# Roboy/gym-roboy

Hardware: AMD Instinct MI355X
Metric: env-steps/sec, MsjRobot (3-DOF/8-tendon) batched rollout (higher is better)
Workload: dtype f32

## Files before the change

gym_roboy_amd/csrc/msj_math.hpp:

```cpp
#pragma once
#include "rtc_compat.hpp"

#if defined(__HIPCC__)
#define RB_HD __host__ __device__ __forceinline__
#else
#define RB_HD inline
#endif


namespace rb {

template <typename T> struct Fast;
template <> struct Fast<double> {
    static RB_HD void sincos(double x, double &s, double &c) { s = ::sin(x); c = ::cos(x); }
    static RB_HD double exp(double x) { return ::exp(x); }
    static RB_HD double exp2(double x) { return ::exp2(x); }
    static RB_HD double rsqrt(double x) { return 1.0 / ::sqrt(x); }
    static RB_HD double rcp(double x) { return 1.0 / x; }
};
template <> struct Fast<float> {
    static RB_HD void sincos(float x, float &s, float &c) {
#if defined(__HIP_DEVICE_COMPILE__)
        s = __sinf(x); c = __cosf(x);
#else
        s = ::sinf(x); c = ::cosf(x);
#endif
    }
    static RB_HD float exp(float x) {
#if defined(__HIP_DEVICE_COMPILE__)
        return __expf(x);
#else
        return ::expf(x);
#endif
    }
    static RB_HD float exp2(float x) {
#if defined(__HIP_DEVICE_COMPILE__)
        return __builtin_amdgcn_exp2f(x);
#else
        return ::exp2f(x);
#endif
    }
    static RB_HD float rsqrt(float x) {
#if defined(__HIP_DEVICE_COMPILE__)
        return __builtin_amdgcn_rsqf(x);
#else
        return 1.0f / ::sqrtf(x);
#endif
    }
    static RB_HD float rcp(float x) {
#if defined(__HIP_DEVICE_COMPILE__)
        return __builtin_amdgcn_rcpf(x);
#else
        return 1.0f / x;
#endif
    }
};

template <typename T> RB_HD T tmin(T a, T b) {
#if defined(__HIP_DEVICE_COMPILE__)
    if constexpr (std::is_same<T, float>::value) return __builtin_fminf(a, b);
#endif
    return a < b ? a : b;
}
template <typename T> RB_HD T tmax(T a, T b) {
#if defined(__HIP_DEVICE_COMPILE__)
    if constexpr (std::is_same<T, float>::value) return __builtin_fmaxf(a, b);
#endif
    return a > b ? a : b;
}
template <typename T> RB_HD T tclamp(T x, T lo, T hi) {
#if defined(__HIP_DEVICE_COMPILE__)
    if constexpr (std::is_same<T, float>::value) return __builtin_amdgcn_fmed3f(x, lo, hi);
#endif
    return tmin(tmax(x, lo), hi);
}

template <typename T>
struct alignas(64) MsjTendon {
    T A[3];
    T Bv[3];
    T B2[3];
    T ab2;
    T il0s;
    T elcs;
    T ksg;
    T fmaxv;
    T pad[2];
};

template <typename T>
struct TendonUnits {
    T lc;
    T vl0;
    T fmax;
    T pad;
};

template <typename T>
struct TendonReading { T length, rate, activation, force; };

template <typename T, int NT>
struct MsjConst {
    MsjTendon<T> ten[NT];
    T IO[6];
    T mc[3];
    T g[3];
    T arm[3], damp[3], qlo[3], qhi[3], qdmax[3];
    T kps;
    T pe_k2s;
    T inv_pe_den;
    T fv_c1l, fv_c2l;
    T fv_c2s;
    T fv_k;
    T h;
    int32_t nsub;
    int32_t simple;
    int32_t nt;
};

template <typename T, int NT>
struct SpArray {
    const T *v;
    RB_HD T operator()(int k) const { return v[k]; }
};

struct NominalBody {
    template <typename T> RB_HD T mass(T x) const { return x; }
    template <typename T> RB_HD T damping(int, T x) const { return x; }
};

template <typename T, int NT>
struct MsjModel {
    using C = MsjConst<T, NT>;

    struct Frame {
        T s0, c0, s1, c1, s2, c2;
        T r00, r01, r02, r10, r11, r12, r20, r21, r22;
        T wx, wy, wz;
    };

    static RB_HD Frame frame(const T q[3], const T qd[3]) {
        Frame f;
        Fast<T>::sincos(q[0], f.s0, f.c0);
        Fast<T>::sincos(q[1], f.s1, f.c1);
        Fast<T>::sincos(q[2], f.s2, f.c2);
        f.r00 = f.c1 * f.c2; f.r01 = -f.c1 * f.s2; f.r02 = f.s1;
        f.r10 = f.c0 * f.s2 + f.s0 * f.s1 * f.c2; f.r11 = f.c0 * f.c2 - f.s0 * f.s1 * f.s2; f.r12 = -f.s0 * f.c1;
        f.r20 = f.s0 * f.s2 - f.c0 * f.s1 * f.c2; f.r21 = f.s0 * f.c2 + f.c0 * f.s1 * f.s2; f.r22 = f.c0 * f.c1;
        f.wx = f.r00 * qd[0] + f.s2 * qd[1];
        f.wy = f.r01 * qd[0] + f.c2 * qd[1];
        f.wz = f.r02 * qd[0] + qd[2];
        return f;
    }

    static RB_HD void tendon(const C &c, const Frame &f, const MsjTendon<T> &t, T u, T &tx, T &ty, T &tz) {
        const T ax = f.r00 * t.A[0] + f.r10 * t.A[1] + f.r20 * t.A[2];
        const T ay = f.r01 * t.A[0] + f.r11 * t.A[1] + f.r21 * t.A[2];
        const T az = f.r02 * t.A[0] + f.r12 * t.A[1] + f.r22 * t.A[2];
        const T d2 = ax * t.B2[0] + (ay * t.B2[1] + (az * t.B2[2] + t.ab2));
        const T mx = ay * t.Bv[2] - az * t.Bv[1];
        const T my = az * t.Bv[0] - ax * t.Bv[2];
        const T mz = ax * t.Bv[1] - ay * t.Bv[0];
        tendon_force(c, f, t, u, d2, mx, my, mz, tx, ty, tz);
    }

    static RB_HD void tendon_force(const C &c, const Frame &f, const MsjTendon<T> &t, T u, T d2, T mx, T my, T mz,
                                   T &tx, T &ty, T &tz) {
        const T inv = Fast<T>::rsqrt(d2);
        const T v = (f.wx * mx + f.wy * my + f.wz * mz) * inv;
        const T es = (d2 * inv) * t.il0s + t.elcs;
        const T act = tclamp(c.kps * es - u, T(0), T(1));
        const T fl = Fast<T>::exp2(-(es * es));
        const T vp = tmax(v, T(0)), p = tclamp(v + T(1), T(0), T(1));
        const T num = c.fv_c1l * vp + p;
        const T den = c.fv_c2l * vp + (c.fv_c2s * p + c.fv_k);
        const T rden = Fast<T>::rcp(den);
        const T fpe = tmax(Fast<T>::exp2(c.pe_k2s * es) * c.inv_pe_den - c.inv_pe_den, T(0));
        const T Fs = (t.fmaxv * inv) * ((act * fl) * num * rden + fpe);
        tx -= Fs * mx; ty -= Fs * my; tz -= Fs * mz;
    }

    static RB_HD TendonReading<T> tendon_state(const C &c, const Frame &f, const MsjTendon<T> &t, const TendonUnits<T> &pu, T u) {
        return tendon_state_sel(c, f, t, pu, u, true);
    }
    static RB_HD TendonReading<T> tendon_state_sel(const C &c, const Frame &f, const MsjTendon<T> &t, const TendonUnits<T> &pu, T u,
                                                   bool want_force) {
        const T ax = f.r00 * t.A[0] + f.r10 * t.A[1] + f.r20 * t.A[2];
        const T ay = f.r01 * t.A[0] + f.r11 * t.A[1] + f.r21 * t.A[2];
        const T az = f.r02 * t.A[0] + f.r12 * t.A[1] + f.r22 * t.A[2];
        const T d2 = ax * t.B2[0] + (ay * t.B2[1] + (az * t.B2[2] + t.ab2));
        const T mx = ay * t.Bv[2] - az * t.Bv[1];
        const T my = az * t.Bv[0] - ax * t.Bv[2];
        const T mz = ax * t.Bv[1] - ay * t.Bv[0];
        const T inv = Fast<T>::rsqrt(d2);
        const T v = (f.wx * mx + f.wy * my + f.wz * mz) * inv;
        const T dl = d2 * inv;
        const T es = dl * t.il0s + t.elcs;
        const T act = tclamp(c.kps * es - u, T(0), T(1));
        TendonReading<T> r;
        r.length = dl + pu.lc;
        r.rate = v * pu.vl0;
        r.activation = act;
        r.force = T(0);
        if (want_force) {
            const T fl = Fast<T>::exp2(-(es * es));
            const T vp = tmax(v, T(0)), p = tclamp(v + T(1), T(0), T(1));
            const T num = c.fv_c1l * vp + p;
            const T den = c.fv_c2l * vp + (c.fv_c2s * p + c.fv_k);
            const T rden = Fast<T>::rcp(den);
            const T fpe = tmax(Fast<T>::exp2(c.pe_k2s * es) * c.inv_pe_den - c.inv_pe_den, T(0));
            r.force = pu.fmax * ((act * fl) * num * rden + fpe);
        }
        return r;
    }

    static RB_HD MsjTendon<T> scaled_tendon(const MsjTendon<T> &t, T fscale) {
        MsjTendon<T> s = t;
        s.fmaxv = t.fmaxv * fscale;
        return s;
    }

    static RB_HD T prescale(const C &c, int k, T setpoint) { return c.ten[k].ksg * setpoint; }

    template <typename BP> static RB_HD T bmass(const BP *bp, T x) {
        if constexpr (std::is_same<BP, NominalBody>::value) return x; else return bp->mass(x);
    }
    template <typename BP> static RB_HD T bdamp(const BP *bp, int j, T x) {
        if constexpr (std::is_same<BP, NominalBody>::value) return x; else return bp->damping(j, x);
    }
    template <typename BP = NominalBody>
    static RB_HD void rigid_body(const C &c, const Frame &f, const T qd[3], T tx, T ty, T tz, T qdd[3], const BP *bp = nullptr) {
        const T r00 = f.r00, r01 = f.r01, r02 = f.r02, s2 = f.s2, c2 = f.c2;
        const T Ixx = bmass(bp, c.IO[0]), Iyy = bmass(bp, c.IO[1]), Izz = bmass(bp, c.IO[2]);
        const T z0x = -f.s1 * c2 * qd[1] - f.c1 * s2 * qd[2];
        const T z0y = f.s1 * s2 * qd[1] - f.c1 * c2 * qd[2];
        const T z0z = f.c1 * qd[1];
        const T bx = z0x * qd[0] + c2 * qd[2] * qd[1];
        const T by = z0y * qd[0] - s2 * qd[2] * qd[1];
        const T bz = z0z * qd[0];
        T m00, m01, m02, m11, m12, m22, vx, vy, vz;
        if (c.simple) {
            const T a0x = Ixx * r00, a0y = Iyy * r01, a0z = Izz * r02;
            const T a1x = Ixx * s2, a1y = Iyy * c2;
            m00 = r00 * a0x + r01 * a0y + r02 * a0z + c.arm[0];
            m01 = s2 * a0x + c2 * a0y;
            m02 = a0z;
            m11 = s2 * a1x + c2 * a1y + c.arm[1];
            m12 = T(0);
            m22 = Izz + c.arm[2];
            const T hx = Ixx * f.wx, hy = Iyy * f.wy, hz = Izz * f.wz;
            const T nx = Ixx * bx + (f.wy * hz - f.wz * hy);
            const T ny = Iyy * by + (f.wz * hx - f.wx * hz);
            const T nz = Izz * bz + (f.wx * hy - f.wy * hx);
            const T k = bmass(bp, c.mc[2]) * c.g[2];
            vx = tx - k * f.r21 - nx;
            vy = ty + k * f.r20 - ny;
            vz = tz - nz;
        } else {
            const T Ixy = bmass(bp, c.IO[3]), Ixz = bmass(bp, c.IO[4]), Iyz = bmass(bp, c.IO[5]);
            const T a0x = Ixx * r00 + Ixy * r01 + Ixz * r02;
            const T a0y = Ixy * r00 + Iyy * r01 + Iyz * r02;
            const T a0z = Ixz * r00 + Iyz * r01 + Izz * r02;
            const T a1x = Ixx * s2 + Ixy * c2;
            const T a1y = Ixy * s2 + Iyy * c2;
            const T a1z = Ixz * s2 + Iyz * c2;
            m00 = r00 * a0x + r01 * a0y + r02 * a0z + c.arm[0];
            m01 = s2 * a0x + c2 * a0y;
            m02 = a0z;
            m11 = s2 * a1x + c2 * a1y + c.arm[1];
            m12 = a1z;
            m22 = Izz + c.arm[2];
            const T hx = a0x * qd[0] + a1x * qd[1] + Ixz * qd[2];
            const T hy = a0y * qd[0] + a1y * qd[1] + Iyz * qd[2];
            const T hz = a0z * qd[0] + a1z * qd[1] + Izz * qd[2];
            const T nx = Ixx * bx + Ixy * by + Ixz * bz + (f.wy * hz - f.wz * hy);
            const T ny = Ixy * bx + Iyy * by + Iyz * bz + (f.wz * hx - f.wx * hz);
            const T nz = Ixz * bx + Iyz * by + Izz * bz + (f.wx * hy - f.wy * hx);
            const T gx = r00 * c.g[0] + f.r10 * c.g[1] + f.r20 * c.g[2];
            const T gy = r01 * c.g[0] + f.r11 * c.g[1] + f.r21 * c.g[2];
            const T gz = r02 * c.g[0] + f.r12 * c.g[1] + f.r22 * c.g[2];
            vx = tx + (bmass(bp, c.mc[1]) * gz - bmass(bp, c.mc[2]) * gy) - nx;
            vy = ty + (bmass(bp, c.mc[2]) * gx - bmass(bp, c.mc[0]) * gz) - ny;
            vz = tz + (bmass(bp, c.mc[0]) * gy - bmass(bp, c.mc[1]) * gx) - nz;
        }
        const T t0 = r00 * vx + r01 * vy + r02 * vz - bdamp(bp, 0, c.damp[0]) * qd[0];
        const T t1 = s2 * vx + c2 * vy - bdamp(bp, 1, c.damp[1]) * qd[1];
        const T t2 = vz - bdamp(bp, 2, c.damp[2]) * qd[2];
        const T k00 = m11 * m22 - m12 * m12;
        const T k01 = m02 * m12 - m01 * m22;
        const T k02 = m01 * m12 - m02 * m11;
        const T k11 = m00 * m22 - m02 * m02;
        const T k12 = m01 * m02 - m00 * m12;
        const T k22 = m00 * m11 - m01 * m01;
        const T idet = Fast<T>::rcp(m00 * k00 + m01 * k01 + m02 * k02);
        qdd[0] = (k00 * t0 + k01 * t1 + k02 * t2) * idet;
        qdd[1] = (k01 * t0 + k11 * t1 + k12 * t2) * idet;
        qdd[2] = (k02 * t0 + k12 * t1 + k22 * t2) * idet;
    }

    template <int UNROLL, typename SP>
    struct AccelAllTendons {
        const C &c;
        const SP &sp;
        RB_HD void operator()(const T q[3], const T qd[3], T qdd[3]) const {
            const Frame f = frame(q, qd);
            T tx = T(0), ty = T(0), tz = T(0);
            if (UNROLL == 0) {
#pragma unroll 1
                for (int k = 0; k < c.nt; ++k) tendon(c, f, c.ten[k], sp(k), tx, ty, tz);
            } else {
                constexpr int U = UNROLL > 0 ? UNROLL : 1;
#pragma unroll U
                for (int k = 0; k < NT; ++k) tendon(c, f, c.ten[k], sp(k), tx, ty, tz);
            }
            rigid_body(c, f, qd, tx, ty, tz, qdd);
        }
    };

    template <int MIRROR> static RB_HD T mirror_sign(int j) { return (j == 2 || j == MIRROR) ? T(-1) : T(1); }
    static RB_HD void half_torque(const C &c, const Frame &f, const T u[4], T &tx, T &ty, T &tz) {
        tx = T(0); ty = T(0); tz = T(0);
#pragma unroll
        for (int k = 0; k < 4; ++k) {
            tendon(c, f, c.ten[k], u[k], tx, ty, tz);
#if defined(__HIP_DEVICE_COMPILE__)
            __builtin_amdgcn_sched_barrier(0);
#endif
        }
    }
    template <int MIRROR>
    static RB_HD void mirror_combine(T &tx, T &ty, T &tz, T px, T py, T pz) {
        tx = MIRROR == 0 ? tx - px : tx + px;
        ty = MIRROR == 0 ? ty + py : ty - py;
        tz = tz - pz;
    }

    static RB_HD void sat(const C &c, const T v[3], T out[3]) {
#pragma unroll
        for (int j = 0; j < 3; ++j) out[j] = tclamp(v[j], -c.qdmax[j], c.qdmax[j]);
    }

    static RB_HD bool limit(const C &c, T q[3], T qd[3]) {
        bool ok = true;
#pragma unroll
        for (int j = 0; j < 3; ++j) {
            const bool over = q[j] > c.qhi[j], under = q[j] < c.qlo[j];
            qd[j] = tclamp(qd[j], under ? T(0) : -c.qdmax[j], over ? T(0) : c.qdmax[j]);
            q[j] = tclamp(q[j], c.qlo[j], c.qhi[j]);
            ok = ok && !(over || under);
        }
        return ok;
    }

    template <int INTEG, typename ACCEL>
    static RB_HD bool integrate(const C &c, T q[3], T qd[3], const ACCEL &accel) {
        bool feasible = true;
        const T h = c.h;
        for (int sub = 0; sub < c.nsub; ++sub) {
            if (INTEG == 0) {
                T a[3];
                accel(q, qd, a);
#pragma unroll
                for (int j = 0; j < 3; ++j) {
                    qd[j] = tclamp(qd[j] + h * a[j], -c.qdmax[j], c.qdmax[j]);
                    q[j] = q[j] + h * qd[j];
                }
            } else {
                T k1q[3], k1v[3], k2q[3], k2v[3], k3q[3], k3v[3], k4q[3], k4v[3], qs[3], vs[3];
                const T hh = T(0.5) * h;
                sat(c, qd, k1q);
                accel(q, k1q, k1v);
#pragma unroll
                for (int j = 0; j < 3; ++j) { qs[j] = q[j] + hh * k1q[j]; vs[j] = qd[j] + hh * k1v[j]; }
                sat(c, vs, k2q);
                accel(qs, k2q, k2v);
#pragma unroll
                for (int j = 0; j < 3; ++j) { qs[j] = q[j] + hh * k2q[j]; vs[j] = qd[j] + hh * k2v[j]; }
                sat(c, vs, k3q);
                accel(qs, k3q, k3v);
#pragma unroll
                for (int j = 0; j < 3; ++j) { qs[j] = q[j] + h * k3q[j]; vs[j] = qd[j] + h * k3v[j]; }
                sat(c, vs, k4q);
                accel(qs, k4q, k4v);
                const T h6 = h * T(1.0 / 6.0);
#pragma unroll
                for (int j = 0; j < 3; ++j) {
                    q[j] = q[j] + h6 * (k1q[j] + T(2) * k2q[j] + T(2) * k3q[j] + k4q[j]);
                    qd[j] = qd[j] + h6 * (k1v[j] + T(2) * k2v[j] + T(2) * k3v[j] + k4v[j]);
                }
            }
            feasible = limit(c, q, qd) && feasible;
        }
        return feasible;
    }

    template <int INTEG, typename ACCEL>
    static RB_HD bool integrate_acc(const C &c, T q[3], T qd[3], const ACCEL &accel) {
        if (INTEG == 0) return integrate<0>(c, q, qd, accel);
        bool feasible = true;
        const T h = c.h, h6 = c.h * T(1.0 / 6.0);
        for (int sub = 0; sub < c.nsub; ++sub) {
            T aq[3] = {T(0), T(0), T(0)}, av[3] = {T(0), T(0), T(0)}, qs[3], vs[3];
#pragma unroll
            for (int j = 0; j < 3; ++j) { qs[j] = q[j]; vs[j] = qd[j]; }
#pragma unroll 1
            for (int stage = 0; stage < 4; ++stage) {
                T kq[3], kv[3];
                sat(c, vs, kq);
                accel(qs, kq, kv);
                const T w = (stage == 0 || stage == 3) ? T(1) : T(2);
                const T a = stage < 2 ? T(0.5) * h : h;
#pragma unroll
                for (int j = 0; j < 3; ++j) {
                    aq[j] += w * kq[j]; av[j] += w * kv[j];
                    qs[j] = q[j] + a * kq[j]; vs[j] = qd[j] + a * kv[j];
                }
            }
#pragma unroll
            for (int j = 0; j < 3; ++j) { q[j] = q[j] + h6 * aq[j]; qd[j] = qd[j] + h6 * av[j]; }
            feasible = limit(c, q, qd) && feasible;
        }
        return feasible;
    }

    struct AccelPinned {
        const C &c;
        const T *u;
        RB_HD void operator()(const T q[3], const T qd[3], T qdd[3]) const {
            const Frame f = frame(q, qd);
            T tx = T(0), ty = T(0), tz = T(0);
#pragma unroll
            for (int k = 0; k < NT; ++k) {
                tendon(c, f, c.ten[k], u[k], tx, ty, tz);
#if defined(__HIP_DEVICE_COMPILE__)
                __builtin_amdgcn_sched_barrier(0);
#endif
            }
            rigid_body(c, f, qd, tx, ty, tz, qdd);
        }
    };

    struct Routing { T d2, mx, my, mz; };
    static RB_HD Routing routing(const Frame &f, const MsjTendon<T> &t) {
        const T ax = f.r00 * t.A[0] + f.r10 * t.A[1] + f.r20 * t.A[2];
        const T ay = f.r01 * t.A[0] + f.r11 * t.A[1] + f.r21 * t.A[2];
        const T az = f.r02 * t.A[0] + f.r12 * t.A[1] + f.r22 * t.A[2];
        Routing r;
        r.d2 = ax * t.B2[0] + (ay * t.B2[1] + (az * t.B2[2] + t.ab2));
        r.mx = ay * t.Bv[2] - az * t.Bv[1];
        r.my = az * t.Bv[0] - ax * t.Bv[2];
        r.mz = ax * t.Bv[1] - ay * t.Bv[0];
        return r;
    }
    struct Strain { T v, es, fl, pe; };
    static RB_HD Strain strain(const C &c, const Frame &f, const MsjTendon<T> &t, const Routing &r, T inv) {
        Strain s;
        s.v = (f.wx * r.mx + f.wy * r.my + f.wz * r.mz) * inv;
        s.es = (r.d2 * inv) * t.il0s + t.elcs;
        s.fl = Fast<T>::exp2(-(s.es * s.es));
        s.pe = Fast<T>::exp2(c.pe_k2s * s.es);
        return s;
    }
    struct Hill { T afn, rden; };
    static RB_HD Hill hill(const C &c, const Strain &s, T u) {
        const T act = tclamp(c.kps * s.es - u, T(0), T(1));
        const T vp = tmax(s.v, T(0)), p = tclamp(s.v + T(1), T(0), T(1));
        const T num = c.fv_c1l * vp + p;
        const T den = c.fv_c2l * vp + (c.fv_c2s * p + c.fv_k);
        Hill h;
        h.rden = Fast<T>::rcp(den);
        h.afn = (act * s.fl) * num;
        return h;
    }
    static RB_HD void torque(const C &c, const MsjTendon<T> &t, const Routing &r, T inv, const Strain &s, const Hill &h,
                             T &tx, T &ty, T &tz) {
        const T fpe = tmax(s.pe * c.inv_pe_den - c.inv_pe_den, T(0));
        const T Fs = (t.fmaxv * inv) * (h.afn * h.rden + fpe);
        tx -= Fs * r.mx; ty -= Fs * r.my; tz -= Fs * r.mz;
    }
    static RB_HD void pin() {
#if defined(__HIP_DEVICE_COMPILE__)
        __builtin_amdgcn_sched_barrier(0);
#endif
    }
    static RB_HD void tendon_pair(const C &c, const Frame &f, const MsjTendon<T> &ta, const MsjTendon<T> &tb, T ua, T ub,
                                  T &tx, T &ty, T &tz) {
        const Routing ra = routing(f, ta);
        pin();
        const T ia = Fast<T>::rsqrt(ra.d2);
        const Routing rb_ = routing(f, tb);
        pin();
        const T ib = Fast<T>::rsqrt(rb_.d2);
        const Strain sa = strain(c, f, ta, ra, ia);
        pin();
        const Hill ha = hill(c, sa, ua);
        const Strain sb = strain(c, f, tb, rb_, ib);
        pin();
        torque(c, ta, ra, ia, sa, ha, tx, ty, tz);
        const Hill hb = hill(c, sb, ub);
        pin();
        torque(c, tb, rb_, ib, sb, hb, tx, ty, tz);
        pin();
    }
    template <typename SP>
    struct AccelPaired {
        const C &c;
        const SP &sp;
        RB_HD void operator()(const T q[3], const T qd[3], T qdd[3]) const {
            static_assert(NT % 2 == 0, "tendons in pairs");
            const Frame f = frame(q, qd);
            T tx = T(0), ty = T(0), tz = T(0);
#pragma unroll
            for (int k = 0; k < NT; k += 2) {
                const T ua = sp(k), ub = sp(k + 1);
                tendon_pair(c, f, c.ten[k], c.ten[k + 1], ua, ub, tx, ty, tz);
            }
            rigid_body(c, f, qd, tx, ty, tz, qdd);
        }
    };
    static constexpr int RS = 9;
    template <int INTEG>
    static RB_HD bool step_rs(const C &c, T q[3], T qd[3], const T u[NT]) {
        return integrate_acc<INTEG>(c, q, qd, AccelPinned{c, u});
    }

    template <int INTEG, typename SP>
    static RB_HD bool step_rs_paired(const C &c, T q[3], T qd[3], const SP &sp) {
        return integrate_acc<INTEG>(c, q, qd, AccelPaired<SP>{c, sp});
    }

    template <int INTEG, int UNROLL, typename SP>
    static RB_HD bool step_sp(const C &c, T q[3], T qd[3], const SP &sp) {
        return integrate<INTEG>(c, q, qd, AccelAllTendons<UNROLL, SP>{c, sp});
    }

    template <int INTEG, int UNROLL = NT>
    static RB_HD bool step(const C &c, T q[3], T qd[3], const T sp[NT]) {
        T u[NT];
#pragma unroll
        for (int k = 0; k < NT; ++k) u[k] = prescale(c, k, sp[k]);
        const SpArray<T, NT> src{u};
        return step_sp<INTEG, UNROLL>(c, q, qd, src);
    }
};

}
```

Before: 20.11 billion.

## Share rotated tendon anchor products across tendons via compile-time plan

Adds a compile-time SharePlan that detects tendons whose anchor coordinates match or are negations of each other. It reuses the partial rotation-times-anchor products (r1*A1 and r0*A0 + r1*A1) across those tendons instead of recomputing the full 3x3 rotation of each anchor. Routing is refactored through a callable so the shared variant plugs into the same pair pipeline. Anchor constants are pinned in VGPRs and contraction is disabled on one product so the shared terms stay bitwise consistent. The cost is a new templated path that keeps prefix arrays live, which may raise register pressure.

```diff
diff --git a/gym_roboy_amd/csrc/msj_math.hpp b/gym_roboy_amd/csrc/msj_math.hpp
--- a/gym_roboy_amd/csrc/msj_math.hpp
+++ b/gym_roboy_amd/csrc/msj_math.hpp
@@ -485,10 +485,15 @@
     }
     static RB_HD void tendon_pair(const C &c, const Frame &f, const MsjTendon<T> &ta, const MsjTendon<T> &tb, T ua, T ub,
                                   T &tx, T &ty, T &tz) {
-        const Routing ra = routing(f, ta);
+        tendon_pair_routed(c, f, ta, tb, ua, ub, tx, ty, tz, [&] { return routing(f, ta); }, [&] { return routing(f, tb); });
+    }
+    template <typename RA, typename RB>
+    static RB_HD void tendon_pair_routed(const C &c, const Frame &f, const MsjTendon<T> &ta, const MsjTendon<T> &tb, T ua, T ub,
+                                         T &tx, T &ty, T &tz, const RA &route_a, const RB &route_b) {
+        const Routing ra = route_a();
         pin();
         const T ia = Fast<T>::rsqrt(ra.d2);
-        const Routing rb_ = routing(f, tb);
+        const Routing rb_ = route_b();
         pin();
         const T ib = Fast<T>::rsqrt(rb_.d2);
         const Strain sa = strain(c, f, ta, ra, ia);
@@ -518,6 +523,111 @@
             rigid_body(c, f, qd, tx, ty, tz, qdd);
         }
     };
+    struct SharePlan {
+        int ip[NT];
+        bool ip_neg[NT];
+        int ps[NT];
+        bool ps_neg[NT];
+        int a2[NT];
+        int n_ip, n_ps;
+        int ops;
+    };
+    static constexpr SharePlan share_plan(const C &c) {
+        SharePlan p{};
+        for (int k = 0; k < NT; ++k) {
+            const T a0 = c.ten[k].A[0], a1 = c.ten[k].A[1];
+            p.ip[k] = k; p.ip_neg[k] = false; p.ps[k] = k; p.ps_neg[k] = false; p.a2[k] = k;
+            for (int j = k - 1; j >= 0 && a1 != T(0); --j) {
+                const T b1 = c.ten[j].A[1];
+                if (b1 == a1 || b1 == -a1) { p.ip[k] = j; p.ip_neg[k] = b1 != a1; }
+            }
+            for (int j = k - 1; j >= 0 && a1 != T(0) && a0 != T(0); --j) {
+                const T b0 = c.ten[j].A[0], b1 = c.ten[j].A[1];
+                if ((b0 == a0 && b1 == a1) || (b0 == -a0 && b1 == -a1)) { p.ps[k] = j; p.ps_neg[k] = b1 != a1; }
+            }
+            for (int j = k - 1; j >= 0; --j)
+                if (p.ps_neg[j] && c.ten[j].A[2] == c.ten[k].A[2]) p.a2[k] = j;
+            p.n_ip += p.ip[k] == k;
+            p.n_ps += p.ps[k] == k;
+        }
+        p.ops = 3 * (p.n_ip + p.n_ps + NT);
+        return p;
+    }
+    static RB_HD T in_vgpr(T x) {
+#if defined(__HIP_DEVICE_COMPILE__)
+        asm("" : "+v"(x));
+#endif
+        return x;
+    }
+    static RB_HD T product(T x, T y) {
+#if defined(__clang__)
+#pragma clang fp contract(off)
+#endif
+        return x * y;
+    }
+    static RB_HD Routing routing_of(T ax, T ay, T az, const MsjTendon<T> &t) {
+        Routing r;
+        r.d2 = ax * t.B2[0] + (ay * t.B2[1] + (az * t.B2[2] + t.ab2));
+        r.mx = ay * t.Bv[2] - az * t.Bv[1];
+        r.my = az * t.Bv[0] - ax * t.Bv[2];
+        r.mz = ax * t.Bv[1] - ay * t.Bv[0];
+        return r;
+    }
+    template <typename TAB>
+    struct SharedRouting {
+        static constexpr SharePlan PLAN = share_plan(TAB::table());
+        struct Prefixes { T m[NT][3], p[NT][3]; };
+        struct Homes { T a2[NT]; };
+        template <int K = 0>
+        static RB_HD void fill(Homes &h) {
+            if constexpr (K < NT) {
+                if constexpr (PLAN.ps_neg[K] && PLAN.a2[K] == K) h.a2[K] = in_vgpr(T(TAB::table().ten[K].A[2]));
+                fill<K + 1>(h);
+            }
+        }
+        template <int K>
+        static RB_HD Routing routing(const Frame &f, const MsjTendon<T> &t, Prefixes &s, const Homes &h) {
+            constexpr int I = PLAN.ip[K], J = PLAN.ps[K], G = PLAN.a2[K];
+            constexpr bool IN = PLAN.ip_neg[K], JN = PLAN.ps_neg[K];
+            constexpr T A0 = TAB::table().ten[K].A[0], A1 = TAB::table().ten[K].A[1], A2 = TAB::table().ten[K].A[2];
+            const T r0[3] = {f.r00, f.r01, f.r02}, r1[3] = {f.r10, f.r11, f.r12}, r2[3] = {f.r20, f.r21, f.r22};
+            T a[3];
+#pragma unroll
+            for (int j = 0; j < 3; ++j) {
+                if constexpr (I == K) s.m[K][j] = product(r1[j], A1);
+                if constexpr (J == K) s.p[K][j] = r0[j] * A0 + (IN ? -s.m[I][j] : s.m[I][j]);
+                if constexpr (JN) a[j] = -s.p[J][j] + r2[j] * h.a2[G];
+                else a[j] = s.p[J][j] + r2[j] * A2;
+            }
+            return routing_of(a[0], a[1], a[2], t);
+        }
+    };
+    template <typename TAB, typename SP>
+    struct AccelShared {
+        using SR = SharedRouting<TAB>;
+        const C &c;
+        const SP &sp;
+        const typename SR::Homes &h;
+        template <int K>
+        RB_HD void pairs(const Frame &f, typename SR::Prefixes &s, T &tx, T &ty, T &tz) const {
+            if constexpr (K < NT) {
+                const T ua = sp(K), ub = sp(K + 1);
+                tendon_pair_routed(c, f, c.ten[K], c.ten[K + 1], ua, ub, tx, ty, tz,
+                                   [&] { return SR::template routing<K>(f, c.ten[K], s, h); },
+                                   [&] { return SR::template routing<K + 1>(f, c.ten[K + 1], s, h); });
+                pairs<K + 2>(f, s, tx, ty, tz);
+            }
+        }
+        RB_HD void operator()(const T q[3], const T qd[3], T qdd[3]) const {
+            static_assert(NT % 2 == 0, "tendons in pairs");
+            const Frame f = frame(q, qd);
+            T tx = T(0), ty = T(0), tz = T(0);
+            typename SR::Prefixes s;
+            pairs<0>(f, s, tx, ty, tz);
+            rigid_body(c, f, qd, tx, ty, tz, qdd);
+        }
+    };
+
     static constexpr int RS = 9;
     template <int INTEG>
     static RB_HD bool step_rs(const C &c, T q[3], T qd[3], const T u[NT]) {
@@ -529,6 +639,13 @@
         return integrate_acc<INTEG>(c, q, qd, AccelPaired<SP>{c, sp});
     }
 
+    template <int INTEG, typename TAB, typename SP>
+    static RB_HD bool step_rs_shared(const C &c, T q[3], T qd[3], const SP &sp) {
+        typename SharedRouting<TAB>::Homes h;
+        SharedRouting<TAB>::fill(h);
+        return integrate_acc<INTEG>(c, q, qd, AccelShared<TAB, SP>{c, sp, h});
+    }
+
     template <int INTEG, int UNROLL, typename SP>
     static RB_HD bool step_sp(const C &c, T q[3], T qd[3], const SP &sp) {
         return integrate<INTEG>(c, q, qd, AccelAllTendons<UNROLL, SP>{c, sp});
```

After: 19.87 billion. 1.2% lower.
